# SnowCheetos/CassMantle

Measured on AMD Instinct MI355X. Metric: SD-1.5 512^2 50-step images/sec (whole node) + p50 guess-score latency, higher is better.
Workload: dtype bf16; 1 GPU; model=sd15 UNet/VAE/CLIP (512x512, 50 steps pndm, cfg 7.5), global_batch=4, seq_len=4096, parallelism=dp1 (rooms)

## Files before the change

### cassmantle_amd/models/layers.py

```python
from __future__ import annotations

import math
import os
from typing import Optional

import torch
import torch.nn as nn

from .. import ops


def _param(shape, std, gen: Optional[torch.Generator], dtype) -> nn.Parameter:
    t = torch.randn(*shape, generator=gen, dtype=torch.float32) * std
    return nn.Parameter(t.to(dtype), requires_grad=False)


def _zeros(shape, dtype) -> nn.Parameter:
    return nn.Parameter(torch.zeros(*shape, dtype=dtype), requires_grad=False)


def _ones(shape, dtype) -> nn.Parameter:
    return nn.Parameter(torch.ones(*shape, dtype=dtype), requires_grad=False)


# ... 153 lines not shown
        return self.to_out(o.reshape(B, N, C), residual=residual, row_stats=row_stats)


class CrossAttention(nn.Module):
    def __init__(self, dim: int, ctx_dim: int, heads: int, gen=None, dtype=torch.bfloat16):
        super().__init__()
        self.dim, self.heads = dim, heads
        self.head_dim = dim // heads
        self.to_q = Linear(dim, dim, bias=False, gen=gen, dtype=dtype)
        self.to_kv = Linear(ctx_dim, 2 * dim, bias=False, gen=gen, dtype=dtype)
        self.to_out = Linear(dim, dim, bias=True, gen=gen, dtype=dtype)

    _kv = None
    _kv8 = None

    def forward(self, x, ctx, residual=None, fp8=False, q=None, row_stats=None):
        if q is None:
            q = self.to_q(x)
        B, N = q.shape[0], q.shape[1]
        C = self.dim
        q = q.view(B, N, self.heads, self.head_dim)
        kv8 = None
        if self._kv is not None and self._kv.shape[0] == B:
            kv = self._kv.view(B, self._kv.shape[1], 2, self.heads, self.head_dim)
            kv8 = self._kv8 if fp8 else None
        else:
            kv = self.to_kv(ctx).view(B, ctx.shape[1], 2, self.heads, self.head_dim)
        o = ops.attention(q, kv[:, :, 0], kv[:, :, 1], fp8=fp8, kv8=kv8)
        return self.to_out(o.reshape(B, N, C), residual=residual, row_stats=row_stats)


class GEGLUFeedForward(nn.Module):
    def __init__(self, dim: int, mult: int = 4, gen=None, dtype=torch.bfloat16):
        super().__init__()
        inner = dim * mult
        self.proj_in = Linear(dim, 2 * inner, gen=gen, dtype=dtype)
# ... 5 lines not shown
```

### cassmantle_amd/models/unet.py

```python
from __future__ import annotations

import os
from dataclasses import dataclass, field
from typing import List, Optional, Sequence, Tuple

import torch
import torch.nn as nn

from .. import ops
from .layers import (Conv2d, CrossAttention, GEGLUFeedForward, GroupNorm, LayerNorm, Linear,
                     SelfAttention, StatsArena)


@dataclass
class UNetConfig:
    in_channels: int = 4
    out_channels: int = 4
    block_out_channels: Tuple[int, ...] = (320, 640, 1280, 1280)
    down_attn: Tuple[bool, ...] = (True, True, True, False)
    transformer_depth: Tuple[int, ...] = (1, 1, 1, 1)
    mid_transformer_depth: int = 1
    layers_per_block: int = 2
    heads: Tuple[int, ...] = (8, 8, 8, 8)
    head_dim: Optional[int] = None
# ... 54 lines not shown
        if pair and self.conv_shortcut is None:
            sc = torch.cat(x, dim=-1)
        elif pair:
            cs = self.conv_shortcut
            sc = ops.linear_cat(x[0], x[1], cs.weight.view(cs.cout, cs.cin), cs.bias)
        else:
            sc = self.conv_shortcut(x) if self.conv_shortcut is not None else x
        s2 = arena.take(B, cout) if arena is not None else None
        return self.conv2(h, residual=sc, stats=s2), s2


_LN_FOLD = os.environ.get("CASSMANTLE_LN_FOLD", "1") == "1"
_LN_ROWSTATS = os.environ.get("CASSMANTLE_LN_ROWSTATS", "1") == "1"
_GN_FOLD = os.environ.get("CASSMANTLE_GN_FOLD", "1") == "1"
_FF_ROWSTATS = os.environ.get("CASSMANTLE_FF_ROWSTATS", "1") == "1"


def _row_stats_wanted(x: torch.Tensor) -> bool:
    return (_LN_ROWSTATS and x.device.type == "cuda" and ops.get_mode() == "hip" and ops.LN_FOLD_MODE == 1
            and x.shape[-1] not in (320, 640) and x.shape[-1] % 8 == 0 and x.numel() // x.shape[-1] >= 1024)


_FP8_KV_EPILOGUE = os.environ.get("CASSMANTLE_FP8_KV_EPILOGUE", "1") == "1"


class BasicTransformerBlock(nn.Module):
    def __init__(self, dim: int, heads: int, ctx_dim: int, gen, dtype):
        super().__init__()
        self.norm1 = LayerNorm(dim, 1e-5, dtype)
        self.attn1 = SelfAttention(dim, heads, gen=gen, dtype=dtype)
# ... 7 lines not shown
    def _fold_sources(self):
        return ((self.norm1, self.attn1.to_qkv), (self.norm2, self.attn2.to_q), (self.norm3, self.ff.proj_in))

    def folds(self):
        key = tuple((n.weight._version, None if n.bias is None else n.bias._version, l.weight._version,
                     None if l.bias is None else l.bias._version) for n, l in self._fold_sources())
        buf = self._buffers.get("fold0_w")
        if buf is None or self._fold_key != key or buf.device != self.norm1.weight.device:
            for i, (n, l) in enumerate(self._fold_sources()):
                for tag, t in zip(("w", "s", "b"), ops.ln_fold(n.weight, n.bias, l.weight, l.bias)):
                    self.register_buffer(f"fold{i}_{tag}", t, persistent=False)
            self._fold_key = key
        return tuple((self._buffers[f"fold{i}_w"], self._buffers[f"fold{i}_s"], self._buffers[f"fold{i}_b"])
                     for i in range(3))

    def forward(self, x, ctx, fp8=False, arena: Optional[StatsArena] = None, xrs=None, out_stats=False):
        if _LN_FOLD and x.device.type == "cuda" and ops.get_mode() == "hip":
            f = self.folds()
            n1, n2, n3 = self.norm1, self.norm2, self.norm3
            want = arena is not None and _row_stats_wanted(x)
            rows = x.numel() // x.shape[-1]
            kv8 = None
            if fp8 and _FP8_KV_EPILOGUE and ops.kv8_ok(x, self.attn1.head_dim):
                kv8 = ops.kv8_image(x.shape[0], x.shape[1], x.shape[2], x.device)
            qkv = ops.ln_linear(x, n1.weight, n1.bias, n1.eps, self.attn1.to_qkv.weight, fold=f[0], kv8=kv8,
                                row_stats=xrs if want else None)
            r2 = arena.take_rows(rows) if want else None
            x = self.attn1(None, residual=x, fp8=fp8, qkv=qkv, kv8=kv8, row_stats=r2)
            q = ops.ln_linear(x, n2.weight, n2.bias, n2.eps, self.attn2.to_q.weight, fold=f[1], row_stats=r2)
            r3 = arena.take_rows(rows) if want else None
            x = self.attn2(None, ctx, residual=x, fp8=fp8, q=q, row_stats=r3)
            h = ops.ln_linear(x, n3.weight, n3.bias, n3.eps, self.ff.proj_in.weight, act="geglu", fold=f[2],
                              row_stats=r3)
            r4 = arena.take_rows(rows) if (want and out_stats and _FF_ROWSTATS) else None
            return self.ff.proj_out(h, residual=x, row_stats=r4), r4
        x = self.attn1(self.norm1(x), residual=x, fp8=fp8)
        x = self.attn2(self.norm2(x), ctx, residual=x, fp8=fp8)
        x = self.ff(self.norm3(x), residual=x)
        return x, None


class Transformer2D(nn.Module):
    def __init__(self, dim: int, heads: int, depth: int, ctx_dim: int, groups: int, gen, dtype):
        super().__init__()
        self.norm = GroupNorm(groups, dim, 1e-6, dtype)
        self.proj_in = Linear(dim, dim, gen=gen, dtype=dtype)
        self.transformer_blocks = nn.ModuleList(
            [BasicTransformerBlock(dim, heads, ctx_dim, gen, dtype) for _ in range(depth)])
        self.proj_out = Linear(dim, dim, gen=gen, dtype=dtype)

    def forward(self, x, ctx, fp8=False, arena: Optional[StatsArena] = None, xs=None):
        B, H, W, C = x.shape
        hrs = None
        if (_GN_FOLD and xs is not None and C == 320 and (H * W) % 256 == 0 and x.device.type == "cuda"
                and ops.get_mode() == "hip"):
            n = self.norm
            h = ops.gn_linear(x.view(B, H * W, C), xs, n.weight, n.bias, n.groups, n.eps, self.proj_in.weight,
                              self.proj_in.bias)
        else:
            h = self.norm(x, stats=xs).view(B, H * W, C)
            hrs = arena.take_rows(B * H * W) if (arena is not None and _LN_FOLD and _row_stats_wanted(h)) else None
            h = self.proj_in(h, row_stats=hrs)
        rs = hrs
        nblk = len(self.transformer_blocks)
        for i, blk in enumerate(self.transformer_blocks):
            h, rs = blk(h, ctx, fp8=fp8, arena=arena, xrs=rs, out_stats=i + 1 < nblk)
        so = arena.take(B, C) if arena is not None else None
        return self.proj_out(h, residual=x.view(B, H * W, C), stats=so).view(B, H, W, C), so


class Downsample(nn.Module):
    def __init__(self, c: int, gen, dtype):
        super().__init__()
        self.conv = Conv2d(c, c, 3, stride=2, padding=1, gen=gen, dtype=dtype)

    def forward(self, x, arena: Optional[StatsArena] = None):
        so = arena.take(x.shape[0], self.conv.cout) if arena is not None else None
        return self.conv(x, stats=so), so


class Upsample(nn.Module):
    def __init__(self, c: int, gen, dtype):
        super().__init__()
# ... 143 lines not shown
        t = t_rep if t_rep is not None else tsteps.float().repeat_interleave(nb)
        rep = None
        if added is not None:
            if rep_ids is not None and ops._use_hip(added["text_embeds"]):
                rep = {"text_embeds": ops.gather_add(added["text_embeds"], rep_ids),
                       "time_ids": added["time_ids_rep"] if "time_ids_rep" in added
                       else added["time_ids"].repeat(E, 1)}
            else:
                rep = {k: v.repeat(E, *([1] * (v.dim() - 1))) for k, v in added.items() if k != "time_ids_rep"}
        temb = self.time_embed(t, rep)
        tb = ops.linear(temb, self._tb_w, self._tb_b)
        return temb.view(E, nb, -1), tb.view(E, nb, -1)

    def forward(self, x: torch.Tensor, t: Optional[torch.Tensor], ctx: torch.Tensor,
                added: Optional[dict] = None, fp8: bool = False, time_cond=None,
                out: Optional[torch.Tensor] = None) -> torch.Tensor:
        if not getattr(self, "_fused", False):
            self.fuse_projections()
        if time_cond is not None:
            temb, tb = time_cond
        else:
            temb = self.time_embed(t, added)
            tb = ops.linear(temb, self._tb_w, self._tb_b)
        ar = self._arena.begin(tuple(x.shape), x)
        B = x.shape[0]
        hs = ar.take(B, self.conv_in.cout)
        h = self.conv_in(x, stats=hs)
        skips = [(h, hs)]
        for blk in self.down:
            for j, res in enumerate(blk.resnets):
                h, hs = res(h, temb, tb, ar, hs)
                if len(blk.attentions):
                    h, hs = blk.attentions[j](h, ctx, fp8, ar, hs)
                skips.append((h, hs))
            if blk.downsampler is not None:
                h, hs = blk.downsampler(h, ar)
                skips.append((h, hs))
        h, hs = self.mid_res1(h, temb, tb, ar, hs)
        h, hs = self.mid_attn(h, ctx, fp8, ar, hs)
        h, hs = self.mid_res2(h, temb, tb, ar, hs)
        for blk in self.up:
            for j, res in enumerate(blk.resnets):
                sk, sks = skips.pop()
                two = hs is not None and sks is not None
                h, hs = res((h, sk), temb, tb, ar, hs if two else None, sks if two else None)
# ... 11 lines not shown
```

### cassmantle_amd/ops/__init__.py

```python
from __future__ import annotations

import math
import os
from typing import List, Optional

import torch

from . import reference as ref
from ._ext import ext, ext_available, ext_error

_MODE = os.environ.get("CASSMANTLE_OPS", "hip").lower()


def set_mode(mode: str) -> None:
    global _MODE
    assert mode in ("hip", "torch")
    _MODE = mode


def get_mode() -> str:
    return _MODE


def _use_hip(t: torch.Tensor) -> bool:
# ... 93 lines not shown
    stats[..., 0] += torch.round(yf.sum(1) * STAT_SCALE[0]).to(torch.int64)
    stats[..., 1] += torch.round((yf * yf).sum(1) * STAT_SCALE[1]).to(torch.int64)


def channel_stats(y: torch.Tensor, stats: torch.Tensor) -> None:
    if _use_hip(y):
        ext().channel_stats(y.contiguous(), stats)
    else:
        channel_stats_ref(y, stats)


def linear(x: torch.Tensor, w: torch.Tensor, bias: Optional[torch.Tensor] = None,
           residual: Optional[torch.Tensor] = None, act: Optional[str] = None,
           stats: Optional[torch.Tensor] = None, out: Optional[torch.Tensor] = None,
           row_stats: Optional[torch.Tensor] = None) -> torch.Tensor:
    if not _use_hip(x):
        if x.device.type == "cuda":
            y = _torch_linear(x, w, bias, residual, act)
        else:
            y = ref.linear(x, w, bias, residual, act)
        if stats is not None:
            channel_stats_ref(y, stats)
        return y if out is None else out.copy_(y)
    K = x.shape[-1]
    x2 = x.reshape(-1, K)
    if not x2.is_contiguous():
        x2 = x2.contiguous()
    N = w.shape[0] // 2 if act in ("geglu", "swiglu") else w.shape[0]
    if out is None:
        out = torch.empty((x2.shape[0], N), device=x.device, dtype=x.dtype)
    else:
        assert out.is_contiguous() and out.dtype == x.dtype and out.numel() == x2.shape[0] * N, "linear: bad out"
    o2 = out.view(x2.shape[0], N)
    r2 = residual.reshape(-1, N) if residual is not None else None
    hw = x2.shape[0] // x.shape[0] if stats is not None else 0
    if row_stats is not None:
        _launch(ext().gemm, x2, w, bias, r2, o2, _ACT[act], stats, hw, row_stats=row_stats)
    else:
        _launch(ext().gemm, x2, w, bias, r2, o2, _ACT[act], stats, hw)
    return out.view(*x.shape[:-1], N)


def gn_linear(x: torch.Tensor, stats: torch.Tensor, gamma: torch.Tensor, beta: torch.Tensor, groups: int,
# ... 346 lines not shown

def set_fp8_attention_variant(variant: Optional[str]) -> None:
    if variant is None:
        ext().set_fp8_attn_variant(0)
        return
    assert variant in FP8_ATTN_VARIANTS, variant
    nq, ns = (int(x) for x in variant.split("x"))
    ext().set_fp8_attn_variant(nq * 10 + ns)


def attention(q: torch.Tensor, k: torch.Tensor, v: torch.Tensor, scale: Optional[float] = None,
              causal: bool = False, kv_lens: Optional[torch.Tensor] = None,
              fp8: bool = False, kv8: Optional[torch.Tensor] = None) -> torch.Tensor:
    d = q.shape[-1]
    scale = scale if scale is not None else 1.0 / math.sqrt(d)
    if not _use_hip(q):
        if q.device.type == "cuda":
            import torch.nn.functional as F
            if k.shape[2] != q.shape[2]:
                g = q.shape[2] // k.shape[2]
                k, v = k.repeat_interleave(g, dim=2), v.repeat_interleave(g, dim=2)
            mask = None
            if kv_lens is not None:
                ar = torch.arange(k.shape[1], device=q.device)
                mask = (ar[None, :] < kv_lens[:, None])[:, None, None, :]
            o = F.scaled_dot_product_attention(q.transpose(1, 2), k.transpose(1, 2), v.transpose(1, 2),
                                               attn_mask=mask, is_causal=causal and mask is None, scale=scale)
            return o.transpose(1, 2)
        return ref.attention(q, k, v, scale, causal, kv_lens)
    B, Nq, H, _ = q.shape
    if d > 160 and d != 512:
        return _attention_gemm(q, k, v, scale, causal, kv_lens)
    out = torch.empty((B, Nq, H, d), device=q.device, dtype=q.dtype)
    use8 = fp8 == "force" or (bool(fp8) and d == 64 and (kv8 is not None or k.shape[1] >= FP8_MIN_KEYS))
    ext().attention(q, k, v, out, float(scale), int(causal), kv_lens, int(use8), kv8 if use8 else None)
    return out


FP8_MIN_KEYS = 256


def _attention_gemm(q, k, v, scale, causal, kv_lens):
    B, Nq, H, d = q.shape
    outs = []
    for h in range(H):
        qh, kh, vh = q[:, :, h], k[:, :, h], v[:, :, h]
        s = torch.empty((B, Nq, k.shape[1]), device=q.device, dtype=torch.float32)
        ext().bmm_nt(qh, kh, s, float(scale))
        p = torch.empty((B, Nq, k.shape[1]), device=q.device, dtype=q.dtype)
# ... 462 lines not shown
```

### cassmantle_amd/ops/csrc/attention.hip

```cpp
#include <atomic>

#include "common.h"
#include "kernels.h"

namespace {

constexpr int KT = 64;

#ifndef ATTN_KBATCH
#define ATTN_KBATCH 1
#endif
#ifndef ATTN_PERMLANE
#define ATTN_PERMLANE 1
#endif
#ifndef ATTN_BRANCHLESS
#define ATTN_BRANCHLESS 0
#endif
#ifndef ATTN_PRIO
#define ATTN_PRIO 1
#endif
#ifndef F8_ONES_SUM
#define F8_ONES_SUM 1
#endif

// ... 36 lines not shown

  const int nqb = (a.Nq + QB - 1) / QB;
  const int bid = xcd_remap(blockIdx.x, gridDim.x);
  const int qb = bid % nqb;
  const int bh = bid / nqb;
  const int h = bh % a.H;
  const int b = bh / a.H;
  const int q0 = qb * QB + wave * 32;
  const int q = q0 + ql;

  int nk = a.Nk;
  if (a.kv_lens) nk = min(nk, a.kv_lens[b]);
  int ntiles = (nk + KT - 1) / KT;
  if (a.causal) ntiles = min(ntiles, (qb * QB + QB + KT - 1) / KT);

  const uint16_t* Qp = a.q + (long long)b * a.q_sb + (long long)h * a.q_sh;
  const int hk = a.group > 1 ? h / a.group : h;
  const uint16_t* Kp = a.k + (long long)b * a.k_sb + (long long)hk * a.k_sh;
  const uint16_t* Vp = a.v + (long long)b * a.v_sb + (long long)hk * a.v_sh;
  const int d = a.d;

  bf16x8_t qf[NKS];
#pragma unroll
  for (int ks = 0; ks < NKS; ++ks) {
    uint4 v = make_uint4(0, 0, 0, 0);
    int d0 = ks * 16 + 8 * hlf;
    if (q < a.Nq && d0 < d) v = *reinterpret_cast<const uint4*>(Qp + (long long)q * a.q_sn + d0);
    float f[8];
    unpack8(v, f);
#pragma unroll
    for (int j = 0; j < 8; ++j) f[j] *= a.scale * 1.4426950408889634f;
// ... 282 lines not shown
  const int wave = tid >> 6;
  const int g = lane >> 4, li = lane & 15;

  const int nqb = (a.Nq + QB - 1) / QB;
  const int bid = xcd_remap(blockIdx.x, gridDim.x);
  const int qblk = bid % nqb;
  const int bh = bid / nqb;
  const int h = bh % a.H;
  const int b = bh / a.H;
  const int q0 = qblk * QB + wave * 32;

  int nk = a.Nk;
  if (a.kv_lens) nk = min(nk, a.kv_lens[b]);
  const int ntiles = (nk + KT - 1) / KT;

  const uint16_t* Qp = a.q + (long long)b * a.q_sb + (long long)h * a.q_sh;
  const int hk = a.group > 1 ? h / a.group : h;
  const uint16_t* Kp = a.k + (long long)b * a.k_sb + (long long)hk * a.k_sh;
  const uint16_t* Vp = a.v + (long long)b * a.v_sb + (long long)hk * a.v_sh;

  const float qs = a.scale * 1.4426950408889634f;
  bf16x8_t qA[2], qB[2];
#pragma unroll
  for (int qb = 0; qb < 2; ++qb) {
    const int q = q0 + 16 * qb + li;
    uint4 v = make_uint4(0, 0, 0, 0), w = make_uint4(0, 0, 0, 0);
    if (q < a.Nq) {
      v = *reinterpret_cast<const uint4*>(Qp + (long long)q * a.q_sn + 8 * g);
      if (g == 0) w = *reinterpret_cast<const uint4*>(Qp + (long long)q * a.q_sn + 32);
    }
    float f[8], e[8];
// ... 698 lines not shown
```

### cassmantle_amd/ops/csrc/bindings.cpp

```cpp
#include <torch/extension.h>
#include <atomic>
#include <ATen/hip/HIPContext.h>
#include <c10/hip/HIPStream.h>
#include <hip/hip_ext.h>

#include "gemm_tiles.h"
#include "kernels.h"

namespace {

hipStream_t cur_stream() { return c10::hip::getCurrentHIPStream().stream(); }

#define CHECK_DEV(t) TORCH_CHECK((t).is_cuda(), #t " must be a GPU tensor")
#define CHECK_BF16(t) TORCH_CHECK((t).scalar_type() == at::kBFloat16, #t " must be bf16")
#define CHECK_CONTIG(t) TORCH_CHECK((t).is_contiguous(), #t " must be contiguous")

const uint16_t* bptr(const at::Tensor& t) { return reinterpret_cast<const uint16_t*>(t.data_ptr()); }
uint16_t* bptr_mut(at::Tensor& t) { return reinterpret_cast<uint16_t*>(t.data_ptr()); }
const uint16_t* opt_bptr(const c10::optional<at::Tensor>& t) {
  if (!t.has_value() || !t->defined()) return nullptr;
  CHECK_DEV(*t);
  CHECK_BF16(*t);
  CHECK_CONTIG(*t);
  return bptr(*t);
// ... 67 lines not shown
          const c10::optional<at::Tensor>& gn_beta, int64_t gn_groups, int64_t gn_hw, double gn_eps) {
  CHECK_DEV(x); CHECK_BF16(x); CHECK_BF16(w); CHECK_CONTIG(w); CHECK_CONTIG(out);
  TORCH_CHECK(x.dim() == 2 && w.dim() == 2 && out.dim() == 2, "gemm: 2-D operands expected");
  TORCH_CHECK(x.stride(1) == 1, "gemm: x rows must be contiguous");
  GemmArgs p;
  p.A = bptr(x); p.W = bptr(w); p.bias = opt_bptr(bias); p.residual = opt_bptr(residual);
  p.M = (int)x.size(0); p.K = (int)x.size(1); p.N = (int)out.size(1); p.Nw = (int)w.size(0);
  p.lda = (int)x.stride(0); p.ldc = p.N; p.act = (int)act;
  TORCH_CHECK(w.size(1) == p.K, "gemm: K mismatch");
  TORCH_CHECK(out.size(0) == p.M, "gemm: M mismatch");
  if (act == 4 || act == 6) {
    TORCH_CHECK(p.Nw == 2 * p.N && p.K % 8 == 0 && p.N % 4 == 0, "geglu/swiglu: W must be [2N,K], K%8==0, N%4==0");
  } else {
    TORCH_CHECK(p.Nw == p.N, "gemm: N mismatch");
  }
  if (residual.has_value() && residual->defined()) TORCH_CHECK(residual->numel() == out.numel(), "gemm: residual shape");
  if (out.scalar_type() == at::kFloat) {
    p.out_f32 = 1;
  } else {
    CHECK_BF16(out);
  }
  p.C = out.data_ptr();
  if (kv8.has_value() && kv8->defined()) {
    CHECK_DEV(*kv8); CHECK_CONTIG(*kv8);
    TORCH_CHECK(kv8->scalar_type() == at::kByte && kv8_ntok > 0 && kv8_ntok % 64 == 0 && p.M % kv8_ntok == 0 &&
                    kv8_hk > 0 && kv8_col0 % 8 == 0 && kv8_col0 + 128 * kv8_hk == p.N && act == 0 &&
                    !p.out_f32 && !(residual.has_value() && residual->defined()) && !(stats.has_value() && stats->defined()),
                "gemm kv8: uint8 image, 64-aligned tokens per image, K|V heads ending the output, plain epilogue");
    TORCH_CHECK(kv8->numel() == 2LL * p.M * kv8_hk * 64, "gemm kv8: image size");
    p.kv8 = kv8->data_ptr<uint8_t>();
    p.kv8_col0 = (int)kv8_col0; p.kv8_ntok = (int)kv8_ntok; p.kv8_hk = (int)kv8_hk;
// ... 347 lines not shown
void attention_fp8_pack(const at::Tensor& k, const at::Tensor& v, const c10::optional<at::Tensor>& kv_lens,
                        at::Tensor& kv8) {
  at::Tensor out = at::empty({1, 1, 1, k.size(3)}, k.options());
  AttnArgs a = attn_args(k, k, v, out, 1.0, 0, kv_lens);
  TORCH_CHECK(a.d == 64, "fp8 attention: head dim 64 only");
  const int Hk = (int)k.size(2);
  TORCH_CHECK(kv8.is_cuda() && kv8.scalar_type() == at::kByte && kv8.is_contiguous() &&
                  kv8.numel() == attention_fp8_bytes(a.B, a.Nk, Hk), "kv8: contiguous uint8 of attention_fp8_bytes");
  launch_attention_fp8_pack(a, Hk, kv8.data_ptr<uint8_t>(), cur_stream());
}

void attention(const at::Tensor& q, const at::Tensor& k, const at::Tensor& v, at::Tensor& out, double scale,
               int64_t causal, const c10::optional<at::Tensor>& kv_lens, int64_t fp8,
               const c10::optional<at::Tensor>& kv8) {
  AttnArgs a = attn_args(q, k, v, out, scale, causal, kv_lens);
  if (a.d == 512) {
    const long long wsb = attention_d512_workspace(a);
    at::Tensor ws;
    if (wsb > 0) ws = at::empty({wsb / 4}, q.options().dtype(at::kFloat));
    launch_attention_d512(a, wsb > 0 ? ws.data_ptr<float>() : nullptr, cur_stream());
    return;
  }
  if (fp8 && a.d == 64) {
    const int Hk = (int)k.size(2);
    if (kv8.has_value() && kv8->defined()) {
      TORCH_CHECK(kv8->is_cuda() && kv8->scalar_type() == at::kByte &&
                      kv8->numel() == attention_fp8_bytes(a.B, a.Nk, Hk), "kv8 does not match K/V");
      launch_attention_fp8(a, Hk, kv8->data_ptr<uint8_t>(), cur_stream(), true);
      return;
    }
// ... 584 lines not shown
```

### cassmantle_amd/ops/csrc/common.h

```cpp
#pragma once
#include <hip/hip_runtime.h>
#include <stdint.h>

typedef __attribute__((ext_vector_type(8))) __bf16 bf16x8_t;
typedef __attribute__((ext_vector_type(4))) __bf16 bf16x4_t;
typedef __attribute__((ext_vector_type(4))) short s16x4_t;
typedef __attribute__((ext_vector_type(4))) float f32x4_t;
typedef __attribute__((ext_vector_type(16))) float f32x16_t;
typedef __attribute__((ext_vector_type(4))) int i32x4_t;

#define CM_DEVICE __device__ __forceinline__

CM_DEVICE float bf2f(uint16_t u) { return __uint_as_float(((uint32_t)u) << 16); }

typedef __attribute__((ext_vector_type(2))) __bf16 bf16x2_t;

CM_DEVICE uint16_t f2bf(float f) { return __builtin_bit_cast(uint16_t, (__bf16)f); }

CM_DEVICE uint32_t pack2(float a, float b) {
  bf16x2_t v = {(__bf16)a, (__bf16)b};
  return __builtin_bit_cast(uint32_t, v);
}

CM_DEVICE uint32_t f8x4(float a, float b, float c, float d) {
// ... 18 lines not shown
  if (rel < C) {
    const long long bh = (long long)b * p.kv8_hk + (rel >> 6);
    *reinterpret_cast<uint32_t*>(p.kv8 + (bh * p.kv8_ntok + key) * 64 + (rel & 63)) = w;
  } else {
    const long long B = p.M / p.kv8_ntok;
    uint8_t* V8t = p.kv8 + B * p.kv8_hk * p.kv8_ntok * 64;
    const long long bh = (long long)b * p.kv8_hk + ((rel - C) >> 6);
    const long long col = (key & ~63) + f8_slot(key & 63);
    uint8_t* dst = V8t + (bh * 64 + ((rel - C) & 63)) * p.kv8_ntok + col;
#pragma unroll
    for (int e = 0; e < 4; ++e) dst[(long long)e * p.kv8_ntok] = (uint8_t)(w >> (8 * e));
  }
  return true;
}


CM_DEVICE void unpack8(const uint4& v, float* f) {
  f[0] = __uint_as_float(v.x << 16); f[1] = __uint_as_float(v.x & 0xffff0000u);
  f[2] = __uint_as_float(v.y << 16); f[3] = __uint_as_float(v.y & 0xffff0000u);
  f[4] = __uint_as_float(v.z << 16); f[5] = __uint_as_float(v.z & 0xffff0000u);
  f[6] = __uint_as_float(v.w << 16); f[7] = __uint_as_float(v.w & 0xffff0000u);
}

CM_DEVICE uint4 pack8(const float* f) {
  uint4 v;
  v.x = pack2(f[0], f[1]); v.y = pack2(f[2], f[3]);
  v.z = pack2(f[4], f[5]); v.w = pack2(f[6], f[7]);
  return v;
}

// ... 95 lines not shown
```

### cassmantle_amd/ops/csrc/gemm.hip

```cpp
#include <stdio.h>
#include <stdlib.h>

#include <atomic>
#include <mutex>
#include <string>
#include <unordered_map>

#include "common.h"
#include "gemm_tiles.h"
#include "kernels.h"

void gemm_c0_buf_launch(const GemmArgs& p, float* ws, hipStream_t s);
void gemm_c0_launch(const GemmArgs& p, float* ws, hipStream_t s);
void gemm_c1_launch(const GemmArgs& p, float* ws, hipStream_t s);
void gemm_c2_buf_launch(const GemmArgs& p, float* ws, hipStream_t s);
void gemm_c2_launch(const GemmArgs& p, float* ws, hipStream_t s);
void gemm_c3_launch(const GemmArgs& p, float* ws, hipStream_t s);
void gemm_pp_c0_launch(const GemmArgs& p, float* ws, hipStream_t s);
void gemm_pp_c2_launch(const GemmArgs& p, float* ws, hipStream_t s);

namespace {

constexpr int BK = 64;

// ... 35 lines not shown
      if (iy < 0 || iy >= Hv) continue;
      for (int kx = 0; kx < p.ksize; ++kx) {
        int ix = ox * p.stride - p.pad + kx;
        if (ix < 0 || ix >= Wv) continue;
        int sy = p.upsample ? iy >> 1 : iy, sx = p.upsample ? ix >> 1 : ix;
        const uint16_t* a = A + (((long long)b * p.IH + sy) * p.IW + sx) * p.Cin;
        const uint16_t* w = W + (ky * p.ksize + kx) * p.Cin;
        for (int c = 0; c < p.Cin; ++c) s += bf2f(a[c]) * bf2f(w[c]);
      }
    }
  }
  float o = s * p.alpha;
  if (p.bias) o += bf2f(p.bias[n]);
  if (p.chan_bias) o += bf2f(p.chan_bias[(long long)(m / (p.Ho * p.Wo)) * (p.ldcb ? p.ldcb : p.N) + n]);
  o = apply_act(o, p.act);
  if (p.residual) o += bf2f(p.residual[(long long)m * p.ldc + n]);
  if (p.out_f32)
    reinterpret_cast<float*>(p.C)[(long long)batch * p.sC + (long long)m * p.ldc + n] = o;
  else
    reinterpret_cast<uint16_t*>(p.C)[(long long)batch * p.sC + (long long)m * p.ldc + n] = f2bf(o);
}

bool family_runs(GemmTileFamily f, const GemmArgs& p) {
  if (f == kTileStatic) return true;
  if (f == kTileAreg) return gemm_areg_ok(p);
  if (f == kTilePingPong && (p.N % 8 != 0 || p.ldc % 8 != 0 || (p.ldcb ? p.ldcb : p.N) % 4 != 0)) return false;
  return !p.out_f32 && buf_ok(p) && p.K % BK == 0 && (!p.conv || (!p.upsample && p.Cin % 64 == 0)) && p.N > 16;
}

bool cfg_runs(int cfg, const GemmArgs& p) {
  const GemmTile* t = gemm_tile(cfg);
// ... 173 lines not shown
```

### cassmantle_amd/ops/csrc/gemm_areg.hip

```cpp
#include <stdlib.h>

#include "common.h"
#include "kernels.h"

namespace {

typedef __attribute__((address_space(3))) void lds_void;

CM_DEVICE void areg_blds16(__amdgpu_buffer_rsrc_t rs, uint4* lds_wave_base, int voff, int soff) {
  __builtin_amdgcn_raw_ptr_buffer_load_lds(rs, (lds_void*)lds_wave_base, 16, voff, soff, 0, 0);
}

CM_DEVICE void permlane16_swap_padded(unsigned& a, unsigned& b) {
  asm volatile("s_nop 4\n\tv_permlane16_swap_b32 %0, %1\n\ts_nop 1" : "+v"(a), "+v"(b));
}
CM_DEVICE void permlane32_swap_padded(unsigned& a, unsigned& b) {
  asm volatile("s_nop 4\n\tv_permlane32_swap_b32 %0, %1\n\ts_nop 1" : "+v"(a), "+v"(b));
}
CM_DEVICE float scalar_f(float x) {
  asm volatile("" : "+v"(x));
  return x;
}

CM_DEVICE float sum_row_groups(float v) {
// ... 338 lines not shown
  groups = (nchunks + per - 1) / per;
  const size_t lds = (size_t)RING * BNC * (KS / 2) * 128;
  auto* kfn = &gemm_areg_kernel<KS, TI, RING, RW, GEGLU, LNK, GNK>;
  static const bool once = [&] {
    (void)hipFuncSetAttribute((const void*)kfn, hipFuncAttributeMaxDynamicSharedMemorySize, (int)lds);
    return true;
  }();
  (void)once;
  hipLaunchKernelGGL(kfn, dim3(mblocks, groups), dim3(AR_THREADS), lds, s, p, per);
}

}

bool gemm_areg_ok(const GemmArgs& p) {
  if (p.conv || p.A2 || p.batch != 1 || p.out_f32 || p.ln_rows || p.chan_bias || p.split > 1) return false;
  if (p.ln_rows_fx != nullptr || p.row_stats != nullptr) return false;
  if (p.gn_stats != nullptr) {
    if (p.ln_wsum || is_gated(p.act) || !(p.K == 320 || p.K == 640) || p.gn_hw <= 0 || p.gn_hw % 256 ||
        p.M % p.gn_hw)
      return false;
    if (p.gn_groups <= 0 || p.K % p.gn_groups || p.gn_gamma == nullptr || p.gn_beta == nullptr) return false;
  }
  if (p.ln_wsum && !(p.ln_eps > 0.f)) return false;
  if (!(p.K == 320 || p.K == 640) || p.lda % 8 || p.ldc % 8 || p.N % 8) return false;
  const bool gated = is_gated(p.act);
  const int bnc = p.K == 320 ? 64 : 32;
  if ((gated ? 2 * p.N : p.N) % bnc) return false;
  if (gated && p.stats) return false;
  if (p.stats && (p.stats_hw % 64 != 0)) return false;
  if (((uintptr_t)p.A & 15) || ((uintptr_t)p.C & 7) || ((uintptr_t)p.residual & 7) || ((uintptr_t)p.bias & 7))
    return false;
// ... 26 lines not shown
```

### cassmantle_amd/ops/csrc/gemm_impl.h

```cpp
#pragma once
#include <stdlib.h>

#include "common.h"
#include "gemm_tiles.h"
#include "kernels.h"

#ifndef GEMM_DIAG_APRO
#define GEMM_DIAG_APRO 0
#endif
#ifndef GEMM_FRAG_PREFETCH
#define GEMM_FRAG_PREFETCH 0
#endif

namespace {

__device__ uint4 g_zero_page[4];

constexpr int BK = 64;

CM_DEVICE int swz(int row, int chunk) { return chunk ^ ((row >> 1) & 7); }

#ifndef GEMM_PF_SELF
#define GEMM_PF_SELF 0
#endif
// ... 68 lines not shown
  const int hw = p.Ho * p.Wo;
  const int bimg = (p.chan_bias != nullptr) ? (m / hw) : 0;
  const long long cbs = p.ldcb ? p.ldcb : p.N;
  const bool full = (n + 4 <= p.N) && (p.N % 4 == 0) && (p.ldc % 4 == 0) && (cbs % 4 == 0);
  const long long om = out_row(p, m, batch);
  if (p.ln_rows || p.ln_rows_fx) ln_fold4(p, m, n, o);
#pragma unroll
  for (int r = 0; r < 4; ++r) o[r] *= p.alpha;
  if (full) {
    if (p.bias) add4(o, *reinterpret_cast<const uint2*>(p.bias + n));
    if (p.chan_bias) add4(o, *reinterpret_cast<const uint2*>(p.chan_bias + (long long)bimg * cbs + n));
    if (p.act != ACT_NONE) {
#pragma unroll
      for (int r = 0; r < 4; ++r) o[r] = apply_act(o[r], p.act);
    }
    if (p.residual) add4(o, *reinterpret_cast<const uint2*>(p.residual + om * p.ldc + n));
    if (!OUTF32 && kv8_store4(p, m, n, o)) return;
    if constexpr (OUTF32) {
      float* C = reinterpret_cast<float*>(p.C) + (long long)batch * p.sC + om * p.ldc + n;
      *reinterpret_cast<float4*>(C) = make_float4(o[0], o[1], o[2], o[3]);
    } else {
      uint16_t* C = reinterpret_cast<uint16_t*>(p.C) + (long long)batch * p.sC + om * p.ldc + n;
      *reinterpret_cast<uint2*>(C) = make_uint2(pack2(o[0], o[1]), pack2(o[2], o[3]));
    }
  } else {
#pragma unroll
    for (int r = 0; r < 4; ++r) {
      if (n + r >= p.N) break;
      float v = o[r];
      if (p.bias) v += bf2f(p.bias[n + r]);
      if (p.chan_bias) v += bf2f(p.chan_bias[(long long)bimg * cbs + n + r]);
      v = apply_act(v, p.act);
      if (p.residual) v += bf2f(p.residual[om * p.ldc + n + r]);
      if constexpr (OUTF32)
        reinterpret_cast<float*>(p.C)[(long long)batch * p.sC + om * p.ldc + n + r] = v;
      else
        reinterpret_cast<uint16_t*>(p.C)[(long long)batch * p.sC + om * p.ldc + n + r] = f2bf(v);
    }
  }
}

template <bool OUTF32>
CM_DEVICE void epilogue4_call(const GemmArgs& p, int batch, int m, int n, f32x4_t v) {
  float o[4] = {v[0], v[1], v[2], v[3]};
  epilogue4<OUTF32>(p, batch, m, n, o);
}

CM_DEVICE void gated_epilogue4_call(const GemmArgs& p, int batch, int m, int n, f32x4_t hv, f32x4_t gv) {
  float o[4], hh[4] = {hv[0], hv[1], hv[2], hv[3]}, gg[4] = {gv[0], gv[1], gv[2], gv[3]};
  if (p.ln_rows || p.ln_rows_fx) { ln_fold4(p, m, n, hh); ln_fold4(p, m, p.N + n, gg); }
#pragma unroll
  for (int r = 0; r < 4; ++r) {
    float h = hh[r], g = gg[r];
    if (p.bias) { h += bf2f(p.bias[n + r]); g += bf2f(p.bias[p.N + n + r]); }
    o[r] = gate_f(h, g, p.act);
  }
  uint16_t* C = reinterpret_cast<uint16_t*>(p.C) + (long long)batch * p.sC + (long long)m * p.ldc + n;
  if (p.residual) add4(o, *reinterpret_cast<const uint2*>(p.residual + (long long)m * p.ldc + n));
  *reinterpret_cast<uint2*>(C) = make_uint2(pack2(o[0], o[1]), pack2(o[2], o[3]));
}

template <int BM, int BN, int WM, int WN, bool GEGLU, bool OUTF32, int TI, int TJ, int THREADS, bool SPLIT_DIRECT = false>
CM_DEVICE void tile_epilogue(const GemmArgs& p, f32x4_t (&acc)[TI][TJ], uint4* smem, float* __restrict__ partial,
                             int m0, int n0, int batch, int wm, int wn, int tid, int nsplit, int split_id,
                             bool has_acc = true) {
  const int lane = tid & 63;
  const int fr = lane & 15, fq = lane >> 4;
  if constexpr (!OUTF32) {
    constexpr int OBN = GEGLU ? BN / 2 : BN;
    constexpr int OST = OBN + 8;
    const long long cbs = p.ldcb ? p.ldcb : p.N;
    const bool lds_ok = nsplit == 1 && (p.N % 8 == 0) && (p.ldc % 8 == 0) && (cbs % 4 == 0);
    if (lds_ok) {
// ... 44 lines not shown
              }
            }
            *reinterpret_cast<uint2*>(T + ml * OST + nl) = make_uint2(pack2(o[0], o[1]), pack2(o[2], o[3]));
          }
        }
      }
      }
      __syncthreads();
      constexpr int CPR = OBN / 8;
      uint16_t* Cb = reinterpret_cast<uint16_t*>(p.C) + (long long)batch * p.sC;
      auto finish = [&](int row, int c8) -> uint4 {
        const int m = m0 + row, n = n0 + c8 * 8;
        const long long om = out_row(p, m, batch);
        uint4 v = *reinterpret_cast<const uint4*>(T + row * OST + c8 * 8);
        if (p.residual) {
          const uint4 rv = *reinterpret_cast<const uint4*>(p.residual + om * p.ldc + n);
          float a[8], b[8];
          unpack8(v, a);
          unpack8(rv, b);
#pragma unroll
          for (int e = 0; e < 8; ++e) a[e] += b[e];
          v = pack8(a);
        }
        if (p.kv8 != nullptr && n >= p.kv8_col0) {
          if (n < p.kv8_col0 + 64 * p.kv8_hk) {
            float a[8];
            unpack8(v, a);
            const int rel = n - p.kv8_col0, b = m / p.kv8_ntok, key = m - b * p.kv8_ntok;
            const long long bh = (long long)b * p.kv8_hk + (rel >> 6);
            *reinterpret_cast<uint2*>(p.kv8 + (bh * p.kv8_ntok + key) * 64 + (rel & 63)) =
                make_uint2(f8x4(a[0], a[1], a[2], a[3]), f8x4(a[4], a[5], a[6], a[7]));
// ... 710 lines not shown
```

### cassmantle_amd/ops/csrc/kernels.h

```cpp
#pragma once
#include <hip/hip_runtime.h>
#include <stdint.h>

struct GemmArgs {
  const uint16_t* A = nullptr;
  const uint16_t* W = nullptr;
  const uint16_t* bias = nullptr;
  const uint16_t* residual = nullptr;
  const uint16_t* chan_bias = nullptr;
  int ldcb = 0;
  void* C = nullptr;
  int M = 0, N = 0, K = 0, Nw = 0;
  int lda = 0, ldc = 0, ldw = 0;
  long long sA = 0, sW = 0, sC = 0;
  int batch = 1;
  float alpha = 1.f;
  int act = 0;
  int out_f32 = 0;
  int split = 1;
  int cfg = 0;
  int raster = 0;
  int conv = 0, IH = 0, IW = 0, Cin = 0, Ho = 0, Wo = 0, stride = 1, pad = 0, ksize = 1, upsample = 0;
  int parity = 0;
  const uint16_t* rms_gamma = nullptr;
// ... 29 lines not shown
std::string gemm_last_key();
void gemm_last_plan(int* cfg, int* split);
void launch_gemm(const GemmArgs& p, float* ws, hipStream_t s);

struct AttnArgs {
  const uint16_t* q; const uint16_t* k; const uint16_t* v; uint16_t* o;
  long long q_sb, q_sn, q_sh;
  long long k_sb, k_sn, k_sh;
  long long v_sb, v_sn, v_sh;
  long long o_sb, o_sn, o_sh;
  int B, H, Nq, Nk, d;
  float scale;
  int causal;
  const int* kv_lens;
  int group = 1;
};
void launch_attention(const AttnArgs& a, hipStream_t s);
long long attention_d512_workspace(const AttnArgs& a);
void launch_attention_d512(const AttnArgs& a, float* ws, hipStream_t s);
long long attention_fp8_workspace(const AttnArgs& a, int Hk);
void set_fp8_attn_variant(int v);
void set_attn_d40_variant(int v);
void launch_attention_fp8(const AttnArgs& a, int Hk, uint8_t* ws, hipStream_t s, bool packed = false);
void launch_attention_fp8_pack(const AttnArgs& a, int Hk, uint8_t* ws, hipStream_t s);

void launch_group_norm(const uint16_t* x, const uint16_t* gamma, const uint16_t* beta, uint16_t* y,
                       float* ws, int B, long long S, int C, int G, float eps, int silu, hipStream_t s);
void launch_group_norm_cs(const uint16_t* x, const uint16_t* x2, const long long* stats_a, int Ca, const long long* stats_b,
                          const uint16_t* gamma, const uint16_t* beta, uint16_t* y, int B, long long S, int C,
                          int G, float eps, int silu, hipStream_t s);
// ... 119 lines not shown
```

### cassmantle_amd/ops/csrc/lm.hip

```cpp
#include "common.h"
#include "kernels.h"

namespace {

template <int V>
CM_DEVICE float transpose_reduce(float (&v)[V], int lane, int& idx) {
  idx = 0;
  int c = V;
#pragma unroll
  for (int o = 32; o >= 1; o >>= 1) {
    if (c > 1) {
      const bool up = (lane & o) != 0;
#pragma unroll
      for (int i = 0; i < V / 2; ++i) {
        if (i < c / 2) {
          const float send = up ? v[i] : v[i + c / 2];
          const float keep = up ? v[i + c / 2] : v[i];
          v[i] = keep + __shfl_xor(send, o);
        }
      }
      if (up) idx += c / 2;
      c /= 2;
    } else {
      v[0] += __shfl_xor(v[0], o);
// ... 105 lines not shown
  float o = 0.f;
#pragma unroll
  for (int w = 0; w < GEMV_THREADS / 64; ++w) o += red[w][t];
  o *= scale;
  if constexpr (GATED) {
    float g = 0.f;
#pragma unroll
    for (int w = 0; w < GEMV_THREADS / 64; ++w) g += red[w][GEMV_R * MM + t];
    g *= scale;
    if (p.bias) { o += bf2f(p.bias[n]); g += bf2f(p.bias[p.N + n]); }
    o = gate_f(o, g, p.act);
  } else {
    if (p.bias) o += bf2f(p.bias[n]);
    o = apply_act(o, p.act);
  }
  if (p.residual) o += bf2f(p.residual[(long long)m * p.ldc + n]);
  const long long off = (long long)batch * p.sC + (long long)m * p.ldc + n;
  if (p.out_f32) reinterpret_cast<float*>(p.C)[off] = o;
  else reinterpret_cast<uint16_t*>(p.C)[off] = f2bf(o);
}

template <int MM>
void gemv_launch(const GemmArgs& p, hipStream_t s) {
  if (is_gated(p.act)) {
    constexpr int R = gemv_r<MM, true>();
    hipLaunchKernelGGL((gemv_kernel<MM, true>), dim3((p.N + R - 1) / R, 1, p.batch), dim3(GEMV_THREADS), 0, s, p);
  } else {
    constexpr int R = gemv_r<MM, false>();
    hipLaunchKernelGGL((gemv_kernel<MM, false>), dim3((p.N + R - 1) / R, 1, p.batch), dim3(GEMV_THREADS), 0, s, p);
  }
}
// ... 401 lines not shown
```

### cassmantle_amd/pipeline.py

```python
from __future__ import annotations

import contextlib
import os
import threading
import time
from dataclasses import dataclass
from typing import Dict, List, Optional, Sequence, Tuple

import numpy as np
import torch

from . import ops
from .game.content import ImageGenerator, ImageGenerationError
from .models.schedulers import SchedulePlan, make_plan
from .models.text import CLIP_BIGG, CLIP_L, TINY_CLIP, CLIPTextEncoder, CLIPTextConfig
from .models.unet import SD15_UNET, SDXL_UNET, TINY_UNET, UNet, UNetConfig
from .models.vae import SD_VAE, SDXL_VAE, TINY_VAE, VAEConfig, VAEDecoder
from .utils.tracing import TRACER, span


@dataclass
class PipelineSpec:
    name: str
    unet: UNetConfig
# ... 107 lines not shown
        if len(self.text_encoders) == 1:
            ctx, _ = self.text_encoders[0].encode(texts, self.device, graphs=self.use_graphs and _TEXT_GRAPH)
            return ctx, None
        hs, pooled = [], None
        for enc in self.text_encoders:
            h, p = enc.encode(texts, self.device, output_hidden=-2, graphs=self.use_graphs and _TEXT_GRAPH)
            hs.append(h)
            if p is not None:
                pooled = p
        ctx = ops.concat_last(hs[0], hs[1]) if len(hs) == 2 else torch.cat(hs, dim=-1)
        R = self.spec.resolution
        tid = ops.h2d(torch.tensor([R, R, 0, 0, R, R], dtype=torch.float32).repeat(len(texts), 1), self.device)
        return ctx, {"time_ids": tid, "text_embeds": pooled}

    def _unet_step(self, st: _StepState) -> None:
        eps = self.unet(st.unet_in, None, st.ctx, st.added, fp8=self.fp8, time_cond=(st.temb_cur, st.tb_cur))
        ops.latent_step(eps, st.x, st.hist, st.xs, st.coef, st.step, st.unet_in, st.cfg,
                        rows=[(st.temb_tab, st.temb_cur), (st.tb_tab, st.tb_cur)])
        ops.advance_step(st.step)

    def prepare(self) -> None:
        with self._lock:
            self.unet.prepare()
            self.vae.prepare()
            self._states.clear()

    def _state(self, B: int, ctx: torch.Tensor, plan: SchedulePlan, added) -> _StepState:
        key = (B, self.latent_size, plan.name, plan.evals, float(plan.table[0, 13]), tuple(ctx.shape))
        st = self._states.get(key)
        if st is None:
            h = w = self.latent_size
# ... 160 lines not shown
```

Baseline: 7.769 images/s.

## Share CFG halves through the first down block until cross-attention

With classifier-free guidance the unconditional and conditional halves of the batch carry identical latents and timesteps. Up to the first cross-attention they therefore compute identical activations. The UNet now runs conv_in's consumer resnet and the first transformer's self-attention and Q projection on only half the batch. It then expands to the full batch inside cross-attention, using a query-broadcast index in the attention kernel and a half-row residual index in the GEMM epilogues. This roughly halves the work of the highest-resolution first block, at the cost of extra index arithmetic in the GEMM epilogues and restrictions on the fp8 and d=512 attention paths.

After: 7.831 images/s (median of 6 runs). Within noise of the previous version (+0.8%).

```diff
diff --git a/cassmantle_amd/models/layers.py b/cassmantle_amd/models/layers.py
--- a/cassmantle_amd/models/layers.py
+++ b/cassmantle_amd/models/layers.py
@@ -191,12 +191,13 @@
     _kv = None
     _kv8 = None
 
-    def forward(self, x, ctx, residual=None, fp8=False, q=None, row_stats=None):
+    def forward(self, x, ctx, residual=None, fp8=False, q=None, row_stats=None, shared=False):
         if q is None:
             q = self.to_q(x)
-        B, N = q.shape[0], q.shape[1]
+        N = q.shape[1]
         C = self.dim
-        q = q.view(B, N, self.heads, self.head_dim)
+        q = q.view(q.shape[0], N, self.heads, self.head_dim)
+        B = 2 * q.shape[0] if shared else q.shape[0]
         kv8 = None
         if self._kv is not None and self._kv.shape[0] == B:
             kv = self._kv.view(B, self._kv.shape[1], 2, self.heads, self.head_dim)
diff --git a/cassmantle_amd/models/unet.py b/cassmantle_amd/models/unet.py
--- a/cassmantle_amd/models/unet.py
+++ b/cassmantle_amd/models/unet.py
@@ -92,6 +92,7 @@
 _LN_ROWSTATS = os.environ.get("CASSMANTLE_LN_ROWSTATS", "1") == "1"
 _GN_FOLD = os.environ.get("CASSMANTLE_GN_FOLD", "1") == "1"
 _FF_ROWSTATS = os.environ.get("CASSMANTLE_FF_ROWSTATS", "1") == "1"
+_CFG_SHARE = os.environ.get("CASSMANTLE_CFG_SHARE", "1") == "1"
 
 
 def _row_stats_wanted(x: torch.Tensor) -> bool:
@@ -129,7 +130,8 @@
         return tuple((self._buffers[f"fold{i}_w"], self._buffers[f"fold{i}_s"], self._buffers[f"fold{i}_b"])
                      for i in range(3))
 
-    def forward(self, x, ctx, fp8=False, arena: Optional[StatsArena] = None, xrs=None, out_stats=False):
+    def forward(self, x, ctx, fp8=False, arena: Optional[StatsArena] = None, xrs=None, out_stats=False,
+                shared=False):
         if _LN_FOLD and x.device.type == "cuda" and ops.get_mode() == "hip":
             f = self.folds()
             n1, n2, n3 = self.norm1, self.norm2, self.norm3
@@ -143,14 +145,16 @@
             r2 = arena.take_rows(rows) if want else None
             x = self.attn1(None, residual=x, fp8=fp8, qkv=qkv, kv8=kv8, row_stats=r2)
             q = ops.ln_linear(x, n2.weight, n2.bias, n2.eps, self.attn2.to_q.weight, fold=f[1], row_stats=r2)
+            if shared:
+                rows *= 2
             r3 = arena.take_rows(rows) if want else None
-            x = self.attn2(None, ctx, residual=x, fp8=fp8, q=q, row_stats=r3)
+            x = self.attn2(None, ctx, residual=x, fp8=fp8, q=q, row_stats=r3, shared=shared)
             h = ops.ln_linear(x, n3.weight, n3.bias, n3.eps, self.ff.proj_in.weight, act="geglu", fold=f[2],
                               row_stats=r3)
             r4 = arena.take_rows(rows) if (want and out_stats and _FF_ROWSTATS) else None
             return self.ff.proj_out(h, residual=x, row_stats=r4), r4
         x = self.attn1(self.norm1(x), residual=x, fp8=fp8)
-        x = self.attn2(self.norm2(x), ctx, residual=x, fp8=fp8)
+        x = self.attn2(self.norm2(x), ctx, residual=x, fp8=fp8, shared=shared)
         x = self.ff(self.norm3(x), residual=x)
         return x, None
 
@@ -164,7 +168,7 @@
             [BasicTransformerBlock(dim, heads, ctx_dim, gen, dtype) for _ in range(depth)])
         self.proj_out = Linear(dim, dim, gen=gen, dtype=dtype)
 
-    def forward(self, x, ctx, fp8=False, arena: Optional[StatsArena] = None, xs=None):
+    def forward(self, x, ctx, fp8=False, arena: Optional[StatsArena] = None, xs=None, shared=False):
         B, H, W, C = x.shape
         hrs = None
         if (_GN_FOLD and xs is not None and C == 320 and (H * W) % 256 == 0 and x.device.type == "cuda"
@@ -179,9 +183,10 @@
         rs = hrs
         nblk = len(self.transformer_blocks)
         for i, blk in enumerate(self.transformer_blocks):
-            h, rs = blk(h, ctx, fp8=fp8, arena=arena, xrs=rs, out_stats=i + 1 < nblk)
-        so = arena.take(B, C) if arena is not None else None
-        return self.proj_out(h, residual=x.view(B, H * W, C), stats=so).view(B, H, W, C), so
+            h, rs = blk(h, ctx, fp8=fp8, arena=arena, xrs=rs, out_stats=i + 1 < nblk, shared=shared and i == 0)
+        Bo = 2 * B if shared else B
+        so = arena.take(Bo, C) if arena is not None else None
+        return self.proj_out(h, residual=x.view(B, H * W, C), stats=so).view(Bo, H, W, C), so
 
 
 class Downsample(nn.Module):
@@ -355,7 +360,7 @@
 
     def forward(self, x: torch.Tensor, t: Optional[torch.Tensor], ctx: torch.Tensor,
                 added: Optional[dict] = None, fp8: bool = False, time_cond=None,
-                out: Optional[torch.Tensor] = None) -> torch.Tensor:
+                out: Optional[torch.Tensor] = None, shared_halves: bool = False) -> torch.Tensor:
         if not getattr(self, "_fused", False):
             self.fuse_projections()
         if time_cond is not None:
@@ -363,13 +368,23 @@
         else:
             temb = self.time_embed(t, added)
             tb = ops.linear(temb, self._tb_w, self._tb_b)
-        ar = self._arena.begin(tuple(x.shape), x)
         B = x.shape[0]
+        share = (shared_halves and _CFG_SHARE and x.device.type == "cuda" and ops.get_mode() == "hip"
+                 and B % 2 == 0 and (B // 2 * x.shape[1] * x.shape[2]) % 256 == 0
+                 and len(self.down[0].attentions) > 0
+                 and len(self.down[0].attentions[0].transformer_blocks) > 0)
+        ar = self._arena.begin((tuple(x.shape), share), x)
         hs = ar.take(B, self.conv_in.cout)
         h = self.conv_in(x, stats=hs)
         skips = [(h, hs)]
-        for blk in self.down:
+        for i, blk in enumerate(self.down):
             for j, res in enumerate(blk.resnets):
+                if share and i == 0 and j == 0:
+                    Bh = B // 2
+                    h, hs = res(h[:Bh], temb[:Bh], tb[:Bh], ar, None if hs is None else hs[:Bh])
+                    h, hs = blk.attentions[0](h, ctx, fp8, ar, hs, shared=True)
+                    skips.append((h, hs))
+                    continue
                 h, hs = res(h, temb, tb, ar, hs)
                 if len(blk.attentions):
                     h, hs = blk.attentions[j](h, ctx, fp8, ar, hs)
diff --git a/cassmantle_amd/ops/__init__.py b/cassmantle_amd/ops/__init__.py
--- a/cassmantle_amd/ops/__init__.py
+++ b/cassmantle_amd/ops/__init__.py
@@ -131,7 +131,11 @@
            residual: Optional[torch.Tensor] = None, act: Optional[str] = None,
            stats: Optional[torch.Tensor] = None, out: Optional[torch.Tensor] = None,
            row_stats: Optional[torch.Tensor] = None) -> torch.Tensor:
+    K = x.shape[-1]
+    N = w.shape[0] // 2 if act in ("geglu", "swiglu") else w.shape[0]
     if not _use_hip(x):
+        if residual is not None and residual.numel() * 2 == x.numel() // K * N:
+            residual = residual.reshape(-1, N).repeat(2, 1).reshape(*x.shape[:-1], N)
         if x.device.type == "cuda":
             y = _torch_linear(x, w, bias, residual, act)
         else:
@@ -139,11 +143,9 @@
         if stats is not None:
             channel_stats_ref(y, stats)
         return y if out is None else out.copy_(y)
-    K = x.shape[-1]
     x2 = x.reshape(-1, K)
     if not x2.is_contiguous():
         x2 = x2.contiguous()
-    N = w.shape[0] // 2 if act in ("geglu", "swiglu") else w.shape[0]
     if out is None:
         out = torch.empty((x2.shape[0], N), device=x.device, dtype=x.dtype)
     else:
@@ -520,6 +522,9 @@
               fp8: bool = False, kv8: Optional[torch.Tensor] = None) -> torch.Tensor:
     d = q.shape[-1]
     scale = scale if scale is not None else 1.0 / math.sqrt(d)
+    use8 = fp8 == "force" or (bool(fp8) and d == 64 and (kv8 is not None or k.shape[1] >= FP8_MIN_KEYS))
+    if q.shape[0] * 2 == k.shape[0] and (not _use_hip(q) or d > 160 or use8):
+        q = q.repeat(2, 1, 1, 1)
     if not _use_hip(q):
         if q.device.type == "cuda":
             import torch.nn.functional as F
@@ -537,8 +542,7 @@
     B, Nq, H, _ = q.shape
     if d > 160 and d != 512:
         return _attention_gemm(q, k, v, scale, causal, kv_lens)
-    out = torch.empty((B, Nq, H, d), device=q.device, dtype=q.dtype)
-    use8 = fp8 == "force" or (bool(fp8) and d == 64 and (kv8 is not None or k.shape[1] >= FP8_MIN_KEYS))
+    out = torch.empty((2 * B if B * 2 == k.shape[0] else B, Nq, H, d), device=q.device, dtype=q.dtype)
     ext().attention(q, k, v, out, float(scale), int(causal), kv_lens, int(use8), kv8 if use8 else None)
     return out
 
diff --git a/cassmantle_amd/ops/csrc/attention.hip b/cassmantle_amd/ops/csrc/attention.hip
--- a/cassmantle_amd/ops/csrc/attention.hip
+++ b/cassmantle_amd/ops/csrc/attention.hip
@@ -74,7 +74,7 @@
   int ntiles = (nk + KT - 1) / KT;
   if (a.causal) ntiles = min(ntiles, (qb * QB + QB + KT - 1) / KT);
 
-  const uint16_t* Qp = a.q + (long long)b * a.q_sb + (long long)h * a.q_sh;
+  const uint16_t* Qp = a.q + (long long)(b >= a.q_bper ? b - a.q_bper : b) * a.q_sb + (long long)h * a.q_sh;
   const int hk = a.group > 1 ? h / a.group : h;
   const uint16_t* Kp = a.k + (long long)b * a.k_sb + (long long)hk * a.k_sh;
   const uint16_t* Vp = a.v + (long long)b * a.v_sb + (long long)hk * a.v_sh;
@@ -387,7 +387,7 @@
   if (a.kv_lens) nk = min(nk, a.kv_lens[b]);
   const int ntiles = (nk + KT - 1) / KT;
 
-  const uint16_t* Qp = a.q + (long long)b * a.q_sb + (long long)h * a.q_sh;
+  const uint16_t* Qp = a.q + (long long)(b >= a.q_bper ? b - a.q_bper : b) * a.q_sb + (long long)h * a.q_sh;
   const int hk = a.group > 1 ? h / a.group : h;
   const uint16_t* Kp = a.k + (long long)b * a.k_sb + (long long)hk * a.k_sh;
   const uint16_t* Vp = a.v + (long long)b * a.v_sb + (long long)hk * a.v_sh;
diff --git a/cassmantle_amd/ops/csrc/bindings.cpp b/cassmantle_amd/ops/csrc/bindings.cpp
--- a/cassmantle_amd/ops/csrc/bindings.cpp
+++ b/cassmantle_amd/ops/csrc/bindings.cpp
@@ -105,7 +105,11 @@
   } else {
     TORCH_CHECK(p.Nw == p.N, "gemm: N mismatch");
   }
-  if (residual.has_value() && residual->defined()) TORCH_CHECK(residual->numel() == out.numel(), "gemm: residual shape");
+  if (residual.has_value() && residual->defined()) {
+    TORCH_CHECK(residual->numel() == out.numel() || (p.M % 2 == 0 && residual->numel() * 2 == out.numel()),
+                "gemm: residual shape");
+    if (residual->numel() != out.numel()) p.res_rows = p.M / 2;
+  }
   if (out.scalar_type() == at::kFloat) {
     p.out_f32 = 1;
   } else {
@@ -483,6 +487,13 @@
                int64_t causal, const c10::optional<at::Tensor>& kv_lens, int64_t fp8,
                const c10::optional<at::Tensor>& kv8) {
   AttnArgs a = attn_args(q, k, v, out, scale, causal, kv_lens);
+  if (k.size(0) != q.size(0)) {
+    TORCH_CHECK(k.size(0) == 2 * q.size(0) && v.size(0) == k.size(0) && out.size(0) == k.size(0),
+                "attention: q batch must equal, or be half of, the k / v / out batch");
+    TORCH_CHECK(a.d != 512 && !(fp8 && a.d == 64), "attention: no query broadcast in the d = 512 and fp8 kernels");
+    a.q_bper = a.B;
+    a.B = (int)k.size(0);
+  }
   if (a.d == 512) {
     const long long wsb = attention_d512_workspace(a);
     at::Tensor ws;
diff --git a/cassmantle_amd/ops/csrc/common.h b/cassmantle_amd/ops/csrc/common.h
--- a/cassmantle_amd/ops/csrc/common.h
+++ b/cassmantle_amd/ops/csrc/common.h
@@ -56,6 +56,8 @@
   return true;
 }
 
+template <class Args>
+CM_DEVICE long long res_row(const Args& p, long long om) { return om >= p.res_rows ? om - p.res_rows : om; }
 
 CM_DEVICE void unpack8(const uint4& v, float* f) {
   f[0] = __uint_as_float(v.x << 16); f[1] = __uint_as_float(v.x & 0xffff0000u);
diff --git a/cassmantle_amd/ops/csrc/gemm.hip b/cassmantle_amd/ops/csrc/gemm.hip
--- a/cassmantle_amd/ops/csrc/gemm.hip
+++ b/cassmantle_amd/ops/csrc/gemm.hip
@@ -73,7 +73,7 @@
   if (p.bias) o += bf2f(p.bias[n]);
   if (p.chan_bias) o += bf2f(p.chan_bias[(long long)(m / (p.Ho * p.Wo)) * (p.ldcb ? p.ldcb : p.N) + n]);
   o = apply_act(o, p.act);
-  if (p.residual) o += bf2f(p.residual[(long long)m * p.ldc + n]);
+  if (p.residual) o += bf2f(p.residual[res_row(p, m) * p.ldc + n]);
   if (p.out_f32)
     reinterpret_cast<float*>(p.C)[(long long)batch * p.sC + (long long)m * p.ldc + n] = o;
   else
diff --git a/cassmantle_amd/ops/csrc/gemm_areg.hip b/cassmantle_amd/ops/csrc/gemm_areg.hip
--- a/cassmantle_amd/ops/csrc/gemm_areg.hip
+++ b/cassmantle_amd/ops/csrc/gemm_areg.hip
@@ -376,7 +376,7 @@
 
 bool gemm_areg_ok(const GemmArgs& p) {
   if (p.conv || p.A2 || p.batch != 1 || p.out_f32 || p.ln_rows || p.chan_bias || p.split > 1) return false;
-  if (p.ln_rows_fx != nullptr || p.row_stats != nullptr) return false;
+  if (p.ln_rows_fx != nullptr || p.row_stats != nullptr || p.res_rows != 0) return false;
   if (p.gn_stats != nullptr) {
     if (p.ln_wsum || is_gated(p.act) || !(p.K == 320 || p.K == 640) || p.gn_hw <= 0 || p.gn_hw % 256 ||
         p.M % p.gn_hw)
diff --git a/cassmantle_amd/ops/csrc/gemm_impl.h b/cassmantle_amd/ops/csrc/gemm_impl.h
--- a/cassmantle_amd/ops/csrc/gemm_impl.h
+++ b/cassmantle_amd/ops/csrc/gemm_impl.h
@@ -106,7 +106,7 @@
 #pragma unroll
       for (int r = 0; r < 4; ++r) o[r] = apply_act(o[r], p.act);
     }
-    if (p.residual) add4(o, *reinterpret_cast<const uint2*>(p.residual + om * p.ldc + n));
+    if (p.residual) add4(o, *reinterpret_cast<const uint2*>(p.residual + res_row(p, om) * p.ldc + n));
     if (!OUTF32 && kv8_store4(p, m, n, o)) return;
     if constexpr (OUTF32) {
       float* C = reinterpret_cast<float*>(p.C) + (long long)batch * p.sC + om * p.ldc + n;
@@ -123,7 +123,7 @@
       if (p.bias) v += bf2f(p.bias[n + r]);
       if (p.chan_bias) v += bf2f(p.chan_bias[(long long)bimg * cbs + n + r]);
       v = apply_act(v, p.act);
-      if (p.residual) v += bf2f(p.residual[om * p.ldc + n + r]);
+      if (p.residual) v += bf2f(p.residual[res_row(p, om) * p.ldc + n + r]);
       if constexpr (OUTF32)
         reinterpret_cast<float*>(p.C)[(long long)batch * p.sC + om * p.ldc + n + r] = v;
       else
@@ -148,7 +148,7 @@
     o[r] = gate_f(h, g, p.act);
   }
   uint16_t* C = reinterpret_cast<uint16_t*>(p.C) + (long long)batch * p.sC + (long long)m * p.ldc + n;
-  if (p.residual) add4(o, *reinterpret_cast<const uint2*>(p.residual + (long long)m * p.ldc + n));
+  if (p.residual) add4(o, *reinterpret_cast<const uint2*>(p.residual + res_row(p, m) * p.ldc + n));
   *reinterpret_cast<uint2*>(C) = make_uint2(pack2(o[0], o[1]), pack2(o[2], o[3]));
 }
 
@@ -223,7 +223,7 @@
         const long long om = out_row(p, m, batch);
         uint4 v = *reinterpret_cast<const uint4*>(T + row * OST + c8 * 8);
         if (p.residual) {
-          const uint4 rv = *reinterpret_cast<const uint4*>(p.residual + om * p.ldc + n);
+          const uint4 rv = *reinterpret_cast<const uint4*>(p.residual + res_row(p, om) * p.ldc + n);
           float a[8], b[8];
           unpack8(v, a);
           unpack8(rv, b);
diff --git a/cassmantle_amd/ops/csrc/kernels.h b/cassmantle_amd/ops/csrc/kernels.h
--- a/cassmantle_amd/ops/csrc/kernels.h
+++ b/cassmantle_amd/ops/csrc/kernels.h
@@ -7,6 +7,7 @@
   const uint16_t* W = nullptr;
   const uint16_t* bias = nullptr;
   const uint16_t* residual = nullptr;
+  int res_rows = 0;
   const uint16_t* chan_bias = nullptr;
   int ldcb = 0;
   void* C = nullptr;
@@ -67,6 +68,7 @@
   int causal;
   const int* kv_lens;
   int group = 1;
+  int q_bper = 0;
 };
 void launch_attention(const AttnArgs& a, hipStream_t s);
 long long attention_d512_workspace(const AttnArgs& a);
diff --git a/cassmantle_amd/ops/csrc/lm.hip b/cassmantle_amd/ops/csrc/lm.hip
--- a/cassmantle_amd/ops/csrc/lm.hip
+++ b/cassmantle_amd/ops/csrc/lm.hip
@@ -143,7 +143,7 @@
     if (p.bias) o += bf2f(p.bias[n]);
     o = apply_act(o, p.act);
   }
-  if (p.residual) o += bf2f(p.residual[(long long)m * p.ldc + n]);
+  if (p.residual) o += bf2f(p.residual[res_row(p, m) * p.ldc + n]);
   const long long off = (long long)batch * p.sC + (long long)m * p.ldc + n;
   if (p.out_f32) reinterpret_cast<float*>(p.C)[off] = o;
   else reinterpret_cast<uint16_t*>(p.C)[off] = f2bf(o);
diff --git a/cassmantle_amd/pipeline.py b/cassmantle_amd/pipeline.py
--- a/cassmantle_amd/pipeline.py
+++ b/cassmantle_amd/pipeline.py
@@ -145,7 +145,8 @@
         return ctx, {"time_ids": tid, "text_embeds": pooled}
 
     def _unet_step(self, st: _StepState) -> None:
-        eps = self.unet(st.unet_in, None, st.ctx, st.added, fp8=self.fp8, time_cond=(st.temb_cur, st.tb_cur))
+        eps = self.unet(st.unet_in, None, st.ctx, st.added, fp8=self.fp8, time_cond=(st.temb_cur, st.tb_cur),
+                        shared_halves=st.cfg and st.added is None)
         ops.latent_step(eps, st.x, st.hist, st.xs, st.coef, st.step, st.unet_in, st.cfg,
                         rows=[(st.temb_tab, st.temb_cur), (st.tb_tab, st.tb_cur)])
         ops.advance_step(st.step)
```
